# Zhangwenyao1/DreamVLA

Measured on AMD Instinct MI355X. Metric: train samples/sec (CALVIN ABC->D, seq_len=7), higher is better.
Workload: dtype bf16

## Files before the change

dreamvla_amd/csrc/gemm.hip:

```cpp
#include <stdlib.h>

#include <mutex>
#include "gemm_phase.h"
#include "gemm_skinny.h"

namespace dvla_gemm {
#define DVLA_EXTERN_REG(CF, AT, BT, DBG) extern template void launch_one<CF, AT, BT, DBG>(const GemmKArgs&, int, hipStream_t);
#define DVLA_EXTERN_RING(RC, AT, BT, EPI) extern template void launch_ring_one<RC, AT, BT, EPI>(const GemmKArgs&, int, hipStream_t);
#define DVLA_EXTERN_PHASE(AT, BT, EPI, DBG) extern template void launch_phase_one<AT, BT, EPI, DBG>(const GemmKArgs&, int, hipStream_t);
#include "gemm_inst_list.h"
#undef DVLA_EXTERN_REG
#undef DVLA_EXTERN_RING
#undef DVLA_EXTERN_PHASE
}

using namespace dvla_gemm;
namespace {
struct KsumJob { const float* partial; void* out; int64_t len; int rows; int out_bf16; unsigned main_blocks; };
__device__ __forceinline__ bool ksum_tail(const KsumJob& kj) {
  if (blockIdx.x < kj.main_blocks) return false;
  __shared__ float red[16][16];
  const int cl = threadIdx.x & 15, part = threadIdx.x >> 4;
  const int64_t c = (int64_t)(blockIdx.x - kj.main_blocks) * 16 + cl;
  float s = 0.f;
  if (c < kj.len)
#pragma unroll 4
    for (int r = part; r < kj.rows; r += 16) s += kj.partial[(int64_t)r * kj.len + c];
  red[part][cl] = s;
  __syncthreads();
  if (part == 0 && c < kj.len) {
    float tot = 0.f;
#pragma unroll
    for (int q = 0; q < 16; ++q) tot += red[q][cl];
    if (kj.out_bf16) reinterpret_cast<bf16_t*>(kj.out)[c] = f2bf(tot); else reinterpret_cast<float*>(kj.out)[c] = tot;
  }
  return true;
}
__global__ void splitk_reduce_vec_kernel(const float* __restrict__ ws, void* C, int64_t ldc, int c_f32, int accumulate,
                                         int64_t M, int64_t N, int splits, KsumJob kj) {
  if (ksum_tail(kj)) return;
  const int64_t octs = N >> 3;
  const int64_t idx = (int64_t)blockIdx.x * blockDim.x + threadIdx.x;
  if (idx >= M * octs) return;
  const int64_t m = idx / octs, n = (idx - m * octs) << 3;
  const int64_t MN = M * N;
  const float* src = ws + m * N + n;
  float4 a = make_float4(0.f, 0.f, 0.f, 0.f), b = a;
  for (int k = 0; k < splits; ++k) {
    const float4 x = *reinterpret_cast<const float4*>(src + (int64_t)k * MN);
    const float4 y = *reinterpret_cast<const float4*>(src + (int64_t)k * MN + 4);
    a.x += x.x; a.y += x.y; a.z += x.z; a.w += x.w; b.x += y.x; b.y += y.y; b.z += y.z; b.w += y.w;
  }
  if (c_f32) {
    float* c = reinterpret_cast<float*>(C) + m * ldc + n;
    if (accumulate) {
      const float4 o0 = *reinterpret_cast<const float4*>(c), o1 = *reinterpret_cast<const float4*>(c + 4);
      a.x += o0.x; a.y += o0.y; a.z += o0.z; a.w += o0.w; b.x += o1.x; b.y += o1.y; b.z += o1.z; b.w += o1.w;
    }
    *reinterpret_cast<float4*>(c) = a;
    *reinterpret_cast<float4*>(c + 4) = b;
  } else {
    *reinterpret_cast<uint4*>(reinterpret_cast<bf16_t*>(C) + m * ldc + n) =
        make_uint4(pack2bf(a.x, a.y), pack2bf(a.z, a.w), pack2bf(b.x, b.y), pack2bf(b.z, b.w));
  }
}
struct SplitEpi {
  const void* bias; int bias_f32; int act;
  const bf16_t* residual; int64_t ld_res; int64_t res_rows;
};
__global__ void splitk_reduce_epi_kernel(const float* __restrict__ ws, void* C, int64_t ldc, int c_f32, int64_t M, int64_t N,
                                         int splits, SplitEpi e) {
  const int64_t octs = N >> 3;
  const int64_t idx = (int64_t)blockIdx.x * blockDim.x + threadIdx.x;
  if (idx >= M * octs) return;
  const int64_t m = idx / octs, n = (idx - m * octs) << 3;
  const int64_t MN = M * N;
  const float* src = ws + m * N + n;
  float v[8] = {0.f, 0.f, 0.f, 0.f, 0.f, 0.f, 0.f, 0.f};
  for (int k = 0; k < splits; ++k) {
    const float4 x = *reinterpret_cast<const float4*>(src + (int64_t)k * MN);
    const float4 y = *reinterpret_cast<const float4*>(src + (int64_t)k * MN + 4);
    v[0] += x.x; v[1] += x.y; v[2] += x.z; v[3] += x.w; v[4] += y.x; v[5] += y.y; v[6] += y.z; v[7] += y.w;
  }
  if (e.bias) {
    if (e.bias_f32) {
      const float4 b0 = *reinterpret_cast<const float4*>(reinterpret_cast<const float*>(e.bias) + n);
      const float4 b1 = *reinterpret_cast<const float4*>(reinterpret_cast<const float*>(e.bias) + n + 4);
      v[0] += b0.x; v[1] += b0.y; v[2] += b0.z; v[3] += b0.w; v[4] += b1.x; v[5] += b1.y; v[6] += b1.z; v[7] += b1.w;
    } else {
      const uint4 b = *reinterpret_cast<const uint4*>(reinterpret_cast<const bf16_t*>(e.bias) + n);
      const uint32_t w[4] = {b.x, b.y, b.z, b.w};
#pragma unroll
      for (int i = 0; i < 4; ++i) { v[2 * i] += __uint_as_float(w[i] << 16); v[2 * i + 1] += __uint_as_float(w[i] & 0xffff0000u); }
    }
  }
  act_fwd8(v, e.act);
// ... 109 lines not shown
static std::mutex g_sk_mu;
static int g_streamk = -1;
static bool streamk_enabled() {
  if (g_streamk < 0) { const char* e = getenv("DVLA_GEMM_STREAMK"); g_streamk = (e && e[0] == '0') ? 0 : 1; }
  return g_streamk == 1;
}
static bool sk_scratch(hipStream_t stream, int groups, float** slabs, unsigned** flags) {
  if (!streamk_enabled()) return false;
  int dev = 0;
  if (hipGetDevice(&dev) != hipSuccess) return false;
  std::lock_guard<std::mutex> lk(g_sk_mu);
  for (int i = 0; i < g_sk_n; ++i)
    if (g_sk[i].dev == dev && g_sk[i].stream == stream && g_sk[i].groups >= groups) { *slabs = g_sk[i].slabs; *flags = g_sk[i].flags; return true; }
  if (g_sk_n == 16) return false;
  hipStreamCaptureStatus st = hipStreamCaptureStatusNone;
  if (hipStreamIsCapturing(stream, &st) != hipSuccess) { (void)hipGetLastError(); return false; }
  if (st != hipStreamCaptureStatusNone) return false;
  SkScratch e{dev, stream, nullptr, nullptr, groups};
  if (hipMalloc(reinterpret_cast<void**>(&e.slabs), (size_t)groups * PCfg::BM * PCfg::BN * 4) != hipSuccess) { (void)hipGetLastError(); return false; }
  if (hipMalloc(reinterpret_cast<void**>(&e.flags), (size_t)(groups + 1) * 4) != hipSuccess) { (void)hipGetLastError(); (void)hipFree(e.slabs); return false; }
  if (hipMemsetAsync(e.flags, 0, (size_t)(groups + 1) * 4, stream) != hipSuccess) { (void)hipGetLastError(); (void)hipFree(e.slabs); (void)hipFree(e.flags); return false; }
  g_sk[g_sk_n++] = e;
  *slabs = e.slabs; *flags = e.flags;
  return true;
}
inline int streamk_tiles(int64_t tiles, int cus, bool full = false) {
  if (cus % 16 != 0) return 0;
  const int64_t groups = cus / 16, st = (tiles + 15) / 16;
  if (st < groups || st % groups == 0) return 0;
  if (full) return (int)st;
  const int64_t dp_rounds = st / groups - 1;
  return (int)(st - dp_rounds * groups);
}
void launch_phase(GemmKArgs& a, int combo, int split_k, hipStream_t stream, int stream_k = 0) {
  set_tiles<PCfg::BM, PCfg::BN, PCfg::GH>(a);
  a.sk_tiles = 0;
  if (a.K % PCfg::BKS != 0) {
    if (a.ksum_op != 0) launch_phase_one<true, true, EPI_F32, 128 | 8192>(a, split_k, stream);
    else launch_phase_one<true, true, EPI_F32, 128>(a, split_k, stream);
    return;
  }
  if (a.ksum_op != 0) {
    launch_phase_one<true, true, EPI_F32, 8192>(a, split_k, stream);
    return;
  }
  if (stream_k && split_k == 1 && a.ksum_op == 0) {
    const int groups = num_cus();
    const int r = streamk_tiles((int64_t)a.tiles_m * a.tiles_n, groups, stream_k == 2);
    if (r > 0 && sk_scratch(stream, groups, &a.sk_slabs, &a.sk_flags)) a.sk_tiles = r;
  }
  switch (combo) {
    case 0: launch_phase_epi<false, false>(a, split_k, stream); break;
    case 1: launch_phase_epi<false, true>(a, split_k, stream); break;
    case 2: launch_phase_epi<true, false>(a, split_k, stream); break;
    default: launch_phase_epi<true, true>(a, split_k, stream); break;
  }
}
template <class RC>
bool ring_ok(const GemmKArgs& a, int combo) {
  if (!a.a_vec || !a.b_vec || !a.c_vec || !a.aux_vec || !a.epi_vec) return false;
  if (a.K < RC::BKS || a.K % RC::BKS != 0 || a.k_per_split % RC::BKS != 0 || (a.N & 63) != 0) return false;
  if ((int64_t)((a.M + RC::BM - 1) / RC::BM) * ((a.N + RC::BN - 1) / RC::BN) * a.split_k >= (1ll << 30)) return false;
  if (a.M < RC::BM || a.N < RC::BN) return false;
  if ((combo & 2) && (a.M % RC::BM != 0)) return false;
  if ((combo & 1) && (a.N % RC::BN != 0)) return false;
  const int64_t a_far = (int64_t)(((combo & 2) ? RC::BKS : RC::BM) - 1) * a.lda * 2 + 2 * (int64_t)((combo & 2) ? RC::BM : RC::BKS);
  const int64_t b_far = (int64_t)(((combo & 1) ? RC::BKS : RC::BN) - 1) * a.ldb * 2 + 2 * (int64_t)((combo & 1) ? RC::BN : RC::BKS);
  if (a_far >= (1ll << 32) || b_far >= (1ll << 32)) return false;
  return true;
}

bool phase_tail(const GemmKArgs& a, int combo) {
  return a.K % PCfg::BKS != 0 && combo == 3 && epi_class(a) == EPI_F32 && a.K % 16 == 0 && a.K >= 2 * PCfg::BKS;
}
bool phase_ok(const GemmKArgs& a, int combo) {
  if (phase_tail(a, combo)) {
    GemmKArgs b = a;
    b.K = a.K - a.K % PCfg::BKS;
    if (!ring_ok<PCfg>(b, combo)) return false;
  } else if (!ring_ok<PCfg>(a, combo)) return false;
  const int64_t a_rows = (combo & 2) ? a.K : a.M, b_rows = (combo & 1) ? a.K : a.N;
  return a_rows * a.lda * 2 < (1ll << 32) && b_rows * a.ldb * 2 < (1ll << 32);
}

inline double fill(int64_t tiles, int64_t slots) {
  const int64_t rounds = (tiles + slots - 1) / slots;
  return (double)tiles / (double)(rounds * slots);
}

}

static bool launch_phase_experiment(int idx, GemmKArgs& a, int split_k, hipStream_t stream) {
  switch (idx) {
    case 0: launch_phase_one<false, false, 0, 7424>(a, split_k, stream); return true;
    case 1: launch_phase_one<false, false, 0, 7488>(a, split_k, stream); return true;
    case 2: launch_phase_one<false, false, 0, 3328>(a, split_k, stream); return true;
    case 3: launch_phase_one<false, false, 0, 256>(a, split_k, stream); return true;
    case 4: launch_phase_one<false, false, 0, 32768>(a, split_k, stream); return true;
    case 5: launch_phase_one<false, false, 0, 16384 | 65536>(a, split_k, stream); return true;
    case 6: launch_phase_one<false, false, 0, 16384 | 65536 | 131072>(a, split_k, stream); return true;
    case 7: launch_phase_one<false, false, 0, 16384>(a, split_k, stream); return true;
    default: return false;
  }
}

static int g_last_variant = 0;
extern "C" int dvla_last_gemm_variant(void) { return g_last_variant; }
extern "C" void dvla_set_gemm_variant(int v) { g_gemm_variant = v; }
extern "C" void dvla_set_gemm_schedule(int oversubscribe, int stream_k) {
  if (oversubscribe >= 1) dvla_gemm::gemm_oversubscribe() = oversubscribe > 16 ? 16 : oversubscribe;
  if (stream_k >= 0) g_streamk = stream_k ? 1 : 0;
}

extern "C" void dvla_get_gemm_schedule(int* oversubscribe, int* stream_k) {
  if (oversubscribe) *oversubscribe = dvla_gemm::gemm_oversubscribe();
  if (stream_k) *stream_k = streamk_enabled() ? 1 : 0;
}

extern "C" int64_t dvla_gemm_ksum_partial_rows(int32_t split_k) {
  const int64_t fused = (int64_t)(split_k > 1 ? split_k : 1) * dvla_gemm::KSUM_PARTS * 4, fallback = dvla_colsum_partial_rows();
  return fused > fallback ? fused : fallback;
}

extern "C" int dvla_gemm_bf16(const dvla_gemm_params* q, void* stream_) {
  hipStream_t stream = reinterpret_cast<hipStream_t>(stream_);
  if (!q || !q->A || !q->B || !q->C) return DVLA_ERR_ARG;
  if (q->M < 0 || q->N < 0 || q->K < 0) return DVLA_ERR_ARG;
  if (q->M == 0 || q->N == 0) return DVLA_OK;
  if (q->accumulate && q->c_dtype != DVLA_DT_F32) return DVLA_ERR_ARG;
  if (q->dropout_p < 0.f || q->dropout_p >= 1.f) return DVLA_ERR_ARG;
  const int split_k = q->split_k > 1 ? q->split_k : 1;
  const bool split_epi = split_k > 1 && (q->bias || q->act || q->residual);
  if (split_k > 1) {
    if (!q->workspace || q->preact || q->dact_aux || q->dropout_p > 0.f) return DVLA_ERR_ARG;
    if (split_epi) {
      if (q->accumulate || q->ksum_operand != 0) return DVLA_ERR_ARG;
      const bool c_ok = q->c_dtype == DVLA_DT_F32 ? ((q->ldc % 4 == 0) && aligned(q->C, 16)) : ((q->ldc % 8 == 0) && aligned(q->C, 16));
      if ((q->N & 7) != 0 || !aligned(q->workspace, 16) || !c_ok || (q->bias && !aligned(q->bias, 16)) ||
          (q->residual && !((q->ld_res % 8 == 0) && aligned(q->residual, 16))))
        return DVLA_ERR_UNSUPPORTED;
    }
  }
  if (q->ksum_operand != 0) {
    if ((q->ksum_operand != 1 && q->ksum_operand != 2) || !q->ksum || !q->ksum_workspace) return DVLA_ERR_ARG;
    if (q->ksum_dtype != DVLA_DT_F32 && q->ksum_dtype != DVLA_DT_BF16) return DVLA_ERR_ARG;
  }
  GemmKArgs a;
  a.sk_tiles = 0; a.sk_slabs = nullptr; a.sk_flags = nullptr;
  a.ksum_ws = q->ksum_workspace; a.ksum_op = 0;
  a.ksum_parts = KSUM_PARTS;
  a.a_ln = q->a_layernorm != 0; a.a_ln_eps = q->a_ln_eps;
  a.A = reinterpret_cast<const bf16_t*>(q->A); a.lda = q->lda;
  a.B = reinterpret_cast<const bf16_t*>(q->B); a.ldb = q->ldb;
  a.C = q->C; a.ldc = q->ldc; a.c_f32 = (q->c_dtype == DVLA_DT_F32);
  a.M = q->M; a.N = q->N; a.K = q->K;
  a.bias = q->bias; a.bias_f32 = (q->bias_dtype == DVLA_DT_F32);
  a.act = q->act;
  a.preact = reinterpret_cast<bf16_t*>(q->preact); a.ld_preact = q->ld_preact;
  a.dact_aux = reinterpret_cast<const bf16_t*>(q->dact_aux); a.ld_dact = q->ld_dact; a.dact = q->dact;
  a.has_drop = q->dropout_p > 0.f;
  a.drop_scale = a.has_drop ? 1.0f / (1.0f - q->dropout_p) : 1.0f;
  {
    double thr = (double)q->dropout_p * 4294967296.0;
    a.drop_thr = thr >= 4294967295.0 ? 4294967295u : (uint32_t)thr;
  }
  a.seed_lo = q->seed_lo; a.seed_hi = q->seed_hi;
  a.residual = reinterpret_cast<const bf16_t*>(q->residual); a.ld_res = q->ld_res; a.res_rows = q->res_rows;
  a.accumulate = q->accumulate;
  a.split_k = split_k; a.workspace = reinterpret_cast<float*>(q->workspace);
  {
    int64_t nkt = (q->K + BK - 1) / BK;
    int64_t per = (nkt + split_k - 1) / split_k;
    a.k_per_split = per * BK;
  }
  a.a_vec = (q->lda % 8 == 0) && aligned(q->A, 16);
  a.b_vec = (q->ldb % 8 == 0) && aligned(q->B, 16);
  a.c_vec = a.c_f32 ? ((q->ldc % 4 == 0) && aligned(q->C, 16)) : ((q->ldc % 8 == 0) && aligned(q->C, 16));
  a.aux_vec = 1;
  if (q->preact && !((q->ld_preact % 8 == 0) && aligned(q->preact, 16))) a.aux_vec = 0;
  if (q->dact_aux && !((q->ld_dact % 8 == 0) && aligned(q->dact_aux, 16))) a.aux_vec = 0;
  if (q->residual && !((q->ld_res % 8 == 0) && aligned(q->residual, 16))) a.aux_vec = 0;
  if (split_epi) { a.bias = nullptr; a.act = 0; a.residual = nullptr; }
  a.epi_vec = 1;
  if (q->bias && !aligned(q->bias, 16)) a.epi_vec = 0;
  if (split_k > 1 && ((q->N & 3) != 0 || !aligned(q->workspace, 16))) a.epi_vec = 0;

  const int combo = (q->a_trans ? 2 : 0) | (q->b_trans ? 1 : 0);
  int variant = gemm_variant();
  if (variant >= 100) variant %= 100;
  {
    int choice = 0;
    if (a.a_ln && !(skinny_ok(a, combo, split_k) && skinny_ln_ok(a))) return DVLA_ERR_UNSUPPORTED;
    if ((variant == 0 || variant == 11 || a.a_ln) && skinny_ok(a, combo, split_k)) {
      choice = 11;
    } else if (variant == 0) {
      const double ns = (double)(a.k_per_split < a.K ? a.k_per_split : a.K) / 32.0;
      const int slots = num_cus();
      double best = 1e30;
      auto consider = [&](int c, int64_t bm, int64_t bn, int wg_per_cu, double fixed_us, double stage_us) {
        const int64_t items = ((q->M + bm - 1) / bm) * ((q->N + bn - 1) / bn) * split_k;
        const int64_t rounds = (items + (int64_t)slots * wg_per_cu - 1) / ((int64_t)slots * wg_per_cu);
        const double t = (double)rounds * (fixed_us + stage_us * ns);
        if (t < best) { best = t; choice = c; }
      };
      if (ring_ok<RCfgS>(a, combo)) consider(3, 128, 128, 2, 2.9, 0.58);
      if (ring_ok<RCfgM64>(a, combo)) consider(4, 256, 128, 1, 3.6, 0.49);
      if (ring_ok<RCfgL>(a, combo)) consider(1, 256, 256, 1, 5.8, 0.85);
      if (phase_ok(a, combo)) {
        consider(5, 256, 256, 1, 6.6, 0.775);
        const int64_t tiles = ((q->M + 255) / 256) * ((q->N + 255) / 256);
        if (split_k == 1 && streamk_enabled() && streamk_tiles(tiles, slots) > 0) {
          const double t = (double)tiles / slots * (6.6 + 0.775 * ns) + 18.0;
          if (t < best) { best = t; choice = 6; }
        }
      }
    } else if (variant == 4 && ring_ok<RCfgL>(a, combo)) choice = 1;
    else if (variant == 6 && ring_ok<RCfgS>(a, combo)) choice = 3;
    else if (variant == 7 && ring_ok<RCfgM64>(a, combo)) choice = 4;
    else if (variant == 8 && phase_ok(a, combo)) choice = 5;
    else if (variant == 9 && phase_ok(a, combo)) choice = 6;
    else if (variant == 10 && phase_ok(a, combo)) choice = 7;
    else if (variant > 80 && variant < 90 && combo == 0 && phase_ok(a, combo)) choice = 80 + (variant - 80);
    else if (variant >= 40 && variant < 48 && combo == 0 && phase_ok(a, combo) && epi_class(a) == EPI_P0) choice = variant;
    const bool phase_choice = choice == 5 || choice == 6 || choice == 7;
    const bool ksum_fused = q->ksum_operand != 0 && epi_class(a) == EPI_F32 &&
                            (choice == 1 || choice == 3 || choice == 4 || (phase_choice && combo == 3));
    if (ksum_fused) {
      a.ksum_op = q->ksum_operand;
      if (phase_choice) {
        const int64_t other = q->ksum_operand == 1 ? (q->N + PCfg::BN - 1) / PCfg::BN : (q->M + PCfg::BM - 1) / PCfg::BM;
        a.ksum_parts = KSUM_PARTS * (int)(other < 4 ? other : 4);
      }
    }
    switch (choice) {
      case 1: launch_ring<RCfgL>(a, combo, split_k, stream); break;
      case 3: launch_ring<RCfgS>(a, combo, split_k, stream); break;
      case 4: launch_ring<RCfgM64>(a, combo, split_k, stream); break;
      case 5: launch_phase(a, combo, split_k, stream); break;
      case 6: launch_phase(a, combo, split_k, stream, 1); break;
      case 7: launch_phase(a, combo, split_k, stream, 2); break;
      case 11: launch_skinny(a, stream); break;
      case 81: case 83: case 84: case 85: case 86: case 88: case 89:
        set_tiles<PCfg::BM, PCfg::BN, PCfg::GH>(a);
        if (epi_class(a) != EPI_P0) return DVLA_ERR_UNSUPPORTED;
        if (choice == 81) launch_phase_one<false, false, 0, 1>(a, split_k, stream);
        else if (choice == 83) launch_phase_one<false, false, 0, 3>(a, split_k, stream);
        else if (choice == 84) launch_phase_one<false, false, 0, 4>(a, split_k, stream);
        else if (choice == 85) launch_phase_one<false, false, 0, 16>(a, split_k, stream);
        else if (choice == 86) launch_phase_one<false, false, 0, 32>(a, split_k, stream);
        else if (choice == 88) launch_phase_one<false, false, 0, 16448>(a, split_k, stream);
        else launch_phase_one<false, false, 0, 64>(a, split_k, stream);
        break;
      default:
        if (choice >= 40 && choice < 48) {
          set_tiles<PCfg::BM, PCfg::BN, PCfg::GH>(a);
          a.sk_tiles = 0;
          if (launch_phase_experiment(choice - 40, a, split_k, stream)) break;
        }
        launch_cfg<CfgS>(a, combo, split_k, stream); break;
    }
    g_last_variant = choice == 11 ? 11 : choice == 1 ? 4 : choice == 3 ? 6 : choice == 4 ? 7 : choice == 5 ? 8
                   : (choice == 6 || choice == 7) ? (a.sk_tiles > 0 ? (choice == 6 ? 9 : 10) : 8) : choice >= 80 ? choice : 2;
  }
  int rc = dvla_check_launch();
  if (rc != DVLA_OK) return rc;
  KsumJob kj{nullptr, nullptr, 0, 0, 0, 0xffffffffu};
  if (q->ksum_operand != 0) {
    const int64_t len = q->ksum_operand == 1 ? q->M : q->N;
    if (a.ksum_op != 0) {
      if (split_k > 1) kj = KsumJob{a.ksum_ws, q->ksum, len, split_k * a.ksum_parts, q->ksum_dtype == DVLA_DT_BF16, 0u};
      else rc = dvla_reduce_partial_rows(a.ksum_ws, split_k * a.ksum_parts, len, len, q->ksum, q->ksum_dtype == DVLA_DT_BF16, stream);
    } else {
      const bool kmajor = q->ksum_operand == 1 ? q->a_trans != 0 : q->b_trans != 0;
      if (!kmajor) return DVLA_ERR_UNSUPPORTED;
      rc = dvla_colsum_dt(q->ksum_operand == 1 ? q->A : q->B, q->ksum_operand == 1 ? q->lda : q->ldb, q->K, len, q->ksum,
                          q->ksum_dtype, q->ksum_workspace, stream_);
    }
    if (rc != DVLA_OK) return rc;
  }
  if (split_k > 1) {
    const int64_t total = q->M * q->N;
    const bool vec = (q->N & 7) == 0 && aligned(a.workspace, 16) && aligned(q->C, 16) &&
                     (a.c_f32 ? (q->ldc & 3) == 0 : (q->ldc & 7) == 0);
    const unsigned main_blocks = (unsigned)(((vec ? total / 8 : total) + 255) / 256);
    const unsigned tail_blocks = kj.partial ? (unsigned)((kj.len + 15) / 16) : 0u;
    if (kj.partial) kj.main_blocks = main_blocks;
    if (split_epi) {
      SplitEpi e;
      e.bias = q->bias; e.bias_f32 = q->bias_dtype == DVLA_DT_F32; e.act = q->act;
      e.residual = reinterpret_cast<const bf16_t*>(q->residual); e.ld_res = q->ld_res; e.res_rows = q->res_rows;
      hipLaunchKernelGGL(splitk_reduce_epi_kernel, dim3(main_blocks), dim3(256), 0, stream, a.workspace, q->C, q->ldc, a.c_f32, q->M,
                         q->N, split_k, e);
    } else if (vec)
      hipLaunchKernelGGL(splitk_reduce_vec_kernel, dim3(main_blocks + tail_blocks), dim3(256), 0, stream,
                         a.workspace, q->C, q->ldc, a.c_f32, q->accumulate, q->M, q->N, split_k, kj);
    else
      hipLaunchKernelGGL(splitk_reduce_kernel, dim3(main_blocks + tail_blocks), dim3(256), 0, stream,
                         a.workspace, q->C, q->ldc, a.c_f32, q->accumulate, q->M, q->N, split_k, kj);
    rc = dvla_check_launch();
  }
  return rc;
}
```

dreamvla_amd/csrc/gemm_inst_list.h:

```cpp
DVLA_EXTERN_REG(CfgS, false, false, 0)
DVLA_EXTERN_REG(CfgS, false, true, 0)
DVLA_EXTERN_REG(CfgS, true, false, 0)
DVLA_EXTERN_REG(CfgS, true, true, 0)
DVLA_EXTERN_RING(RCfgL, false, false, 0)
DVLA_EXTERN_RING(RCfgL, false, false, 1)
DVLA_EXTERN_RING(RCfgL, false, false, 2)
DVLA_EXTERN_RING(RCfgL, false, false, 3)
DVLA_EXTERN_RING(RCfgL, false, false, 4)
DVLA_EXTERN_RING(RCfgL, false, false, 5)
DVLA_EXTERN_RING(RCfgL, false, false, 6)
DVLA_EXTERN_RING(RCfgL, false, false, 7)
DVLA_EXTERN_RING(RCfgL, false, true, 0)
DVLA_EXTERN_RING(RCfgL, false, true, 1)
DVLA_EXTERN_RING(RCfgL, false, true, 2)
DVLA_EXTERN_RING(RCfgL, false, true, 3)
DVLA_EXTERN_RING(RCfgL, false, true, 4)
DVLA_EXTERN_RING(RCfgL, false, true, 5)
DVLA_EXTERN_RING(RCfgL, false, true, 6)
DVLA_EXTERN_RING(RCfgL, false, true, 7)
DVLA_EXTERN_RING(RCfgL, true, false, 0)
DVLA_EXTERN_RING(RCfgL, true, false, 1)
DVLA_EXTERN_RING(RCfgL, true, false, 2)
DVLA_EXTERN_RING(RCfgL, true, false, 3)
DVLA_EXTERN_RING(RCfgL, true, false, 4)
// ... 42 lines not shown
DVLA_EXTERN_RING(RCfgS, true, true, 7)
DVLA_EXTERN_RING(RCfgM64, false, false, 0)
DVLA_EXTERN_RING(RCfgM64, false, false, 1)
DVLA_EXTERN_RING(RCfgM64, false, false, 2)
DVLA_EXTERN_RING(RCfgM64, false, false, 3)
DVLA_EXTERN_RING(RCfgM64, false, false, 4)
DVLA_EXTERN_RING(RCfgM64, false, false, 5)
DVLA_EXTERN_RING(RCfgM64, false, false, 6)
DVLA_EXTERN_RING(RCfgM64, false, false, 7)
DVLA_EXTERN_RING(RCfgM64, false, true, 0)
DVLA_EXTERN_RING(RCfgM64, false, true, 1)
DVLA_EXTERN_RING(RCfgM64, false, true, 2)
DVLA_EXTERN_RING(RCfgM64, false, true, 3)
DVLA_EXTERN_RING(RCfgM64, false, true, 4)
DVLA_EXTERN_RING(RCfgM64, false, true, 5)
DVLA_EXTERN_RING(RCfgM64, false, true, 6)
DVLA_EXTERN_RING(RCfgM64, false, true, 7)
DVLA_EXTERN_RING(RCfgM64, true, false, 0)
DVLA_EXTERN_RING(RCfgM64, true, false, 1)
DVLA_EXTERN_RING(RCfgM64, true, false, 2)
DVLA_EXTERN_RING(RCfgM64, true, false, 3)
DVLA_EXTERN_RING(RCfgM64, true, false, 4)
DVLA_EXTERN_RING(RCfgM64, true, false, 5)
DVLA_EXTERN_RING(RCfgM64, true, false, 6)
DVLA_EXTERN_RING(RCfgM64, true, false, 7)
DVLA_EXTERN_RING(RCfgM64, true, true, 0)
DVLA_EXTERN_RING(RCfgM64, true, true, 1)
DVLA_EXTERN_RING(RCfgM64, true, true, 2)
DVLA_EXTERN_RING(RCfgM64, true, true, 3)
DVLA_EXTERN_RING(RCfgM64, true, true, 4)
DVLA_EXTERN_RING(RCfgM64, true, true, 5)
DVLA_EXTERN_RING(RCfgM64, true, true, 6)
DVLA_EXTERN_RING(RCfgM64, true, true, 7)
DVLA_EXTERN_PHASE(false, false, 0, 0)
DVLA_EXTERN_PHASE(false, false, 1, 0)
DVLA_EXTERN_PHASE(false, false, 2, 0)
DVLA_EXTERN_PHASE(false, false, 3, 0)
DVLA_EXTERN_PHASE(false, false, 4, 0)
DVLA_EXTERN_PHASE(false, false, 5, 0)
DVLA_EXTERN_PHASE(false, false, 6, 0)
DVLA_EXTERN_PHASE(false, false, 7, 0)
DVLA_EXTERN_PHASE(false, true, 0, 0)
DVLA_EXTERN_PHASE(false, true, 1, 0)
DVLA_EXTERN_PHASE(false, true, 2, 0)
DVLA_EXTERN_PHASE(false, true, 3, 0)
DVLA_EXTERN_PHASE(false, true, 4, 0)
DVLA_EXTERN_PHASE(false, true, 5, 0)
DVLA_EXTERN_PHASE(false, true, 6, 0)
DVLA_EXTERN_PHASE(false, true, 7, 0)
DVLA_EXTERN_PHASE(true, false, 0, 0)
DVLA_EXTERN_PHASE(true, false, 1, 0)
DVLA_EXTERN_PHASE(true, false, 2, 0)
DVLA_EXTERN_PHASE(true, false, 3, 0)
DVLA_EXTERN_PHASE(true, false, 4, 0)
DVLA_EXTERN_PHASE(true, false, 5, 0)
DVLA_EXTERN_PHASE(true, false, 6, 0)
DVLA_EXTERN_PHASE(true, false, 7, 0)
DVLA_EXTERN_PHASE(true, true, 0, 0)
DVLA_EXTERN_PHASE(true, true, 1, 0)
DVLA_EXTERN_PHASE(true, true, 2, 0)
DVLA_EXTERN_PHASE(true, true, 3, 0)
DVLA_EXTERN_PHASE(true, true, 4, 0)
DVLA_EXTERN_PHASE(true, true, 5, 0)
DVLA_EXTERN_PHASE(true, true, 6, 0)
DVLA_EXTERN_PHASE(true, true, 7, 0)
DVLA_EXTERN_PHASE(true, true, 6, 128)
DVLA_EXTERN_PHASE(true, true, 6, 8192)
DVLA_EXTERN_PHASE(true, true, 6, 8320)
DVLA_EXTERN_PHASE(false, false, 0, 1)
DVLA_EXTERN_PHASE(false, false, 0, 3)
DVLA_EXTERN_PHASE(false, false, 0, 4)
DVLA_EXTERN_PHASE(false, false, 0, 16)
DVLA_EXTERN_PHASE(false, false, 0, 32)
DVLA_EXTERN_PHASE(false, false, 0, 64)
DVLA_EXTERN_PHASE(false, false, 0, 7424)
DVLA_EXTERN_PHASE(false, false, 0, 7488)
DVLA_EXTERN_PHASE(false, false, 0, 3328)
DVLA_EXTERN_PHASE(false, false, 0, 256)
DVLA_EXTERN_PHASE(false, false, 0, 16384)
DVLA_EXTERN_PHASE(false, false, 0, 16448)
DVLA_EXTERN_PHASE(false, false, 0, 32768)
DVLA_EXTERN_PHASE(false, false, 0, 81920)
DVLA_EXTERN_PHASE(false, false, 0, 212992)
```

Measured before the change: 229.4.

## Add 256x128 phase-pipelined persistent GEMM kernel and route heuristic to it

```diff
diff --git a/dreamvla_amd/csrc/gemm.hip b/dreamvla_amd/csrc/gemm.hip
--- a/dreamvla_amd/csrc/gemm.hip
+++ b/dreamvla_amd/csrc/gemm.hip
@@ -2,16 +2,19 @@
 
 #include <mutex>
 #include "gemm_phase.h"
+#include "gemm_phase_h.h"
 #include "gemm_skinny.h"
 
 namespace dvla_gemm {
 #define DVLA_EXTERN_REG(CF, AT, BT, DBG) extern template void launch_one<CF, AT, BT, DBG>(const GemmKArgs&, int, hipStream_t);
 #define DVLA_EXTERN_RING(RC, AT, BT, EPI) extern template void launch_ring_one<RC, AT, BT, EPI>(const GemmKArgs&, int, hipStream_t);
 #define DVLA_EXTERN_PHASE(AT, BT, EPI, DBG) extern template void launch_phase_one<AT, BT, EPI, DBG>(const GemmKArgs&, int, hipStream_t);
+#define DVLA_EXTERN_PHASE_H(AT, BT, EPI, DBG) extern template void launch_phase_h_one<AT, BT, EPI, DBG>(const GemmKArgs&, int, hipStream_t);
 #include "gemm_inst_list.h"
 #undef DVLA_EXTERN_REG
 #undef DVLA_EXTERN_RING
 #undef DVLA_EXTERN_PHASE
+#undef DVLA_EXTERN_PHASE_H
 }
 
 using namespace dvla_gemm;
@@ -287,6 +290,47 @@
   const int64_t a_rows = (combo & 2) ? a.K : a.M, b_rows = (combo & 1) ? a.K : a.N;
   return a_rows * a.lda * 2 < (1ll << 32) && b_rows * a.ldb * 2 < (1ll << 32);
 }
+
+bool phase_h_tail(const GemmKArgs& a, int combo) {
+  return a.K % PCfgH::BKS != 0 && combo == 3 && epi_class(a) == EPI_F32 && a.K % 16 == 0 && a.K >= 2 * PCfgH::BKS;
+}
+bool phase_h_ok(const GemmKArgs& a, int combo) {
+  const int ec = epi_class(a);
+  if (ec == EPI_GEN || combo == 2 || (combo == 3 && ec != EPI_F32)) return false;
+  if (phase_h_tail(a, combo)) {
+    GemmKArgs b = a;
+    b.K = a.K - a.K % PCfgH::BKS;
+    if (!ring_ok<PCfgH>(b, combo)) return false;
+  } else if (!ring_ok<PCfgH>(a, combo)) return false;
+  const int64_t a_rows = (combo & 2) ? a.K : a.M, b_rows = (combo & 1) ? a.K : a.N;
+  return a_rows * a.lda * 2 < (1ll << 32) && b_rows * a.ldb * 2 < (1ll << 32);
+}
+template <bool AT, bool BT>
+void launch_phase_h_epi(const GemmKArgs& a, int split_k, hipStream_t stream) {
+  switch (epi_class(a)) {
+    case EPI_P0: launch_phase_h_one<AT, BT, EPI_P0, 0>(a, split_k, stream); break;
+    case EPI_P_ERF: launch_phase_h_one<AT, BT, EPI_P_ERF, 0>(a, split_k, stream); break;
+    case EPI_P_TANH: launch_phase_h_one<AT, BT, EPI_P_TANH, 0>(a, split_k, stream); break;
+    case EPI_A0: launch_phase_h_one<AT, BT, EPI_A0, 0>(a, split_k, stream); break;
+    case EPI_A_ERF: launch_phase_h_one<AT, BT, EPI_A_ERF, 0>(a, split_k, stream); break;
+    case EPI_A_TANH: launch_phase_h_one<AT, BT, EPI_A_TANH, 0>(a, split_k, stream); break;
+    default: launch_phase_h_one<AT, BT, EPI_F32, 0>(a, split_k, stream); break;
+  }
+}
+void launch_phase_h(GemmKArgs& a, int combo, int split_k, hipStream_t stream) {
+  set_tiles<PCfgH::BM, PCfgH::BN, PCfgH::GH>(a);
+  a.sk_tiles = 0;
+  if (combo == 3) {
+    const bool tail = a.K % PCfgH::BKS != 0;
+    if (a.ksum_op != 0) { if (tail) launch_phase_h_one<true, true, EPI_F32, 128 | 8192>(a, split_k, stream); else launch_phase_h_one<true, true, EPI_F32, 8192>(a, split_k, stream); }
+    else { if (tail) launch_phase_h_one<true, true, EPI_F32, 128>(a, split_k, stream); else launch_phase_h_one<true, true, EPI_F32, 0>(a, split_k, stream); }
+    return;
+  }
+  if (combo == 0) launch_phase_h_epi<false, false>(a, split_k, stream);
+  else launch_phase_h_epi<false, true>(a, split_k, stream);
+}
+
+constexpr double PH_FIXED_US = 4.0, PH_STAGE_US = 0.42;
 
 inline double fill(int64_t tiles, int64_t slots) {
   const int64_t rounds = (tiles + slots - 1) / slots;
@@ -410,6 +454,7 @@
       };
       if (ring_ok<RCfgS>(a, combo)) consider(3, 128, 128, 2, 2.9, 0.58);
       if (ring_ok<RCfgM64>(a, combo)) consider(4, 256, 128, 1, 3.6, 0.49);
+      if (phase_h_ok(a, combo)) consider(8, 256, 128, 1, PH_FIXED_US, PH_STAGE_US);
       if (ring_ok<RCfgL>(a, combo)) consider(1, 256, 256, 1, 5.8, 0.85);
       if (phase_ok(a, combo)) {
         consider(5, 256, 256, 1, 6.6, 0.775);
@@ -421,19 +466,21 @@
       }
     } else if (variant == 4 && ring_ok<RCfgL>(a, combo)) choice = 1;
     else if (variant == 6 && ring_ok<RCfgS>(a, combo)) choice = 3;
-    else if (variant == 7 && ring_ok<RCfgM64>(a, combo)) choice = 4;
+    else if (variant == 7 && phase_h_ok(a, combo)) choice = 8;
+    else if ((variant == 7 || variant == 17) && ring_ok<RCfgM64>(a, combo)) choice = 4;
     else if (variant == 8 && phase_ok(a, combo)) choice = 5;
     else if (variant == 9 && phase_ok(a, combo)) choice = 6;
     else if (variant == 10 && phase_ok(a, combo)) choice = 7;
     else if (variant > 80 && variant < 90 && combo == 0 && phase_ok(a, combo)) choice = 80 + (variant - 80);
     else if (variant >= 40 && variant < 48 && combo == 0 && phase_ok(a, combo) && epi_class(a) == EPI_P0) choice = variant;
-    const bool phase_choice = choice == 5 || choice == 6 || choice == 7;
+    const bool phase_choice = choice == 5 || choice == 6 || choice == 7 || choice == 8;
     const bool ksum_fused = q->ksum_operand != 0 && epi_class(a) == EPI_F32 &&
                             (choice == 1 || choice == 3 || choice == 4 || (phase_choice && combo == 3));
     if (ksum_fused) {
       a.ksum_op = q->ksum_operand;
       if (phase_choice) {
-        const int64_t other = q->ksum_operand == 1 ? (q->N + PCfg::BN - 1) / PCfg::BN : (q->M + PCfg::BM - 1) / PCfg::BM;
+        const int64_t bn = choice == 8 ? PCfgH::BN : PCfg::BN;
+        const int64_t other = q->ksum_operand == 1 ? (q->N + bn - 1) / bn : (q->M + PCfg::BM - 1) / PCfg::BM;
         a.ksum_parts = KSUM_PARTS * (int)(other < 4 ? other : 4);
       }
     }
@@ -444,6 +491,7 @@
       case 5: launch_phase(a, combo, split_k, stream); break;
       case 6: launch_phase(a, combo, split_k, stream, 1); break;
       case 7: launch_phase(a, combo, split_k, stream, 2); break;
+      case 8: launch_phase_h(a, combo, split_k, stream); break;
       case 11: launch_skinny(a, stream); break;
       case 81: case 83: case 84: case 85: case 86: case 88: case 89:
         set_tiles<PCfg::BM, PCfg::BN, PCfg::GH>(a);
@@ -464,7 +512,7 @@
         }
         launch_cfg<CfgS>(a, combo, split_k, stream); break;
     }
-    g_last_variant = choice == 11 ? 11 : choice == 1 ? 4 : choice == 3 ? 6 : choice == 4 ? 7 : choice == 5 ? 8
+    g_last_variant = choice == 11 ? 11 : choice == 1 ? 4 : choice == 3 ? 6 : choice == 4 ? 17 : choice == 8 ? 7 : choice == 5 ? 8
                    : (choice == 6 || choice == 7) ? (a.sk_tiles > 0 ? (choice == 6 ? 9 : 10) : 8) : choice >= 80 ? choice : 2;
   }
   int rc = dvla_check_launch();
diff --git a/dreamvla_amd/csrc/gemm_inst/phaseh_NN_e0.hip b/dreamvla_amd/csrc/gemm_inst/phaseh_NN_e0.hip
--- /dev/null
+++ b/dreamvla_amd/csrc/gemm_inst/phaseh_NN_e0.hip
@@ -0,0 +1,2 @@
+#include "../gemm_phase_h.h"
+namespace dvla_gemm { template void launch_phase_h_one<false, false, 0, 0>(const GemmKArgs&, int, hipStream_t); }
diff --git a/dreamvla_amd/csrc/gemm_inst/phaseh_NN_e1.hip b/dreamvla_amd/csrc/gemm_inst/phaseh_NN_e1.hip
--- /dev/null
+++ b/dreamvla_amd/csrc/gemm_inst/phaseh_NN_e1.hip
@@ -0,0 +1,2 @@
+#include "../gemm_phase_h.h"
+namespace dvla_gemm { template void launch_phase_h_one<false, false, 1, 0>(const GemmKArgs&, int, hipStream_t); }
diff --git a/dreamvla_amd/csrc/gemm_inst/phaseh_NN_e2.hip b/dreamvla_amd/csrc/gemm_inst/phaseh_NN_e2.hip
--- /dev/null
+++ b/dreamvla_amd/csrc/gemm_inst/phaseh_NN_e2.hip
@@ -0,0 +1,2 @@
+#include "../gemm_phase_h.h"
+namespace dvla_gemm { template void launch_phase_h_one<false, false, 2, 0>(const GemmKArgs&, int, hipStream_t); }
diff --git a/dreamvla_amd/csrc/gemm_inst/phaseh_NN_e3.hip b/dreamvla_amd/csrc/gemm_inst/phaseh_NN_e3.hip
--- /dev/null
+++ b/dreamvla_amd/csrc/gemm_inst/phaseh_NN_e3.hip
@@ -0,0 +1,2 @@
+#include "../gemm_phase_h.h"
+namespace dvla_gemm { template void launch_phase_h_one<false, false, 3, 0>(const GemmKArgs&, int, hipStream_t); }
diff --git a/dreamvla_amd/csrc/gemm_inst/phaseh_NN_e4.hip b/dreamvla_amd/csrc/gemm_inst/phaseh_NN_e4.hip
--- /dev/null
+++ b/dreamvla_amd/csrc/gemm_inst/phaseh_NN_e4.hip
@@ -0,0 +1,2 @@
+#include "../gemm_phase_h.h"
+namespace dvla_gemm { template void launch_phase_h_one<false, false, 4, 0>(const GemmKArgs&, int, hipStream_t); }
diff --git a/dreamvla_amd/csrc/gemm_inst/phaseh_NN_e5.hip b/dreamvla_amd/csrc/gemm_inst/phaseh_NN_e5.hip
--- /dev/null
+++ b/dreamvla_amd/csrc/gemm_inst/phaseh_NN_e5.hip
@@ -0,0 +1,2 @@
+#include "../gemm_phase_h.h"
+namespace dvla_gemm { template void launch_phase_h_one<false, false, 5, 0>(const GemmKArgs&, int, hipStream_t); }
diff --git a/dreamvla_amd/csrc/gemm_inst/phaseh_NN_e6.hip b/dreamvla_amd/csrc/gemm_inst/phaseh_NN_e6.hip
--- /dev/null
+++ b/dreamvla_amd/csrc/gemm_inst/phaseh_NN_e6.hip
@@ -0,0 +1,2 @@
+#include "../gemm_phase_h.h"
+namespace dvla_gemm { template void launch_phase_h_one<false, false, 6, 0>(const GemmKArgs&, int, hipStream_t); }
diff --git a/dreamvla_amd/csrc/gemm_inst/phaseh_NT_e0.hip b/dreamvla_amd/csrc/gemm_inst/phaseh_NT_e0.hip
--- /dev/null
+++ b/dreamvla_amd/csrc/gemm_inst/phaseh_NT_e0.hip
@@ -0,0 +1,2 @@
+#include "../gemm_phase_h.h"
+namespace dvla_gemm { template void launch_phase_h_one<false, true, 0, 0>(const GemmKArgs&, int, hipStream_t); }
diff --git a/dreamvla_amd/csrc/gemm_inst/phaseh_NT_e1.hip b/dreamvla_amd/csrc/gemm_inst/phaseh_NT_e1.hip
--- /dev/null
+++ b/dreamvla_amd/csrc/gemm_inst/phaseh_NT_e1.hip
@@ -0,0 +1,2 @@
+#include "../gemm_phase_h.h"
+namespace dvla_gemm { template void launch_phase_h_one<false, true, 1, 0>(const GemmKArgs&, int, hipStream_t); }
diff --git a/dreamvla_amd/csrc/gemm_inst/phaseh_NT_e2.hip b/dreamvla_amd/csrc/gemm_inst/phaseh_NT_e2.hip
--- /dev/null
+++ b/dreamvla_amd/csrc/gemm_inst/phaseh_NT_e2.hip
@@ -0,0 +1,2 @@
+#include "../gemm_phase_h.h"
+namespace dvla_gemm { template void launch_phase_h_one<false, true, 2, 0>(const GemmKArgs&, int, hipStream_t); }
diff --git a/dreamvla_amd/csrc/gemm_inst/phaseh_NT_e3.hip b/dreamvla_amd/csrc/gemm_inst/phaseh_NT_e3.hip
--- /dev/null
+++ b/dreamvla_amd/csrc/gemm_inst/phaseh_NT_e3.hip
@@ -0,0 +1,2 @@
+#include "../gemm_phase_h.h"
+namespace dvla_gemm { template void launch_phase_h_one<false, true, 3, 0>(const GemmKArgs&, int, hipStream_t); }
diff --git a/dreamvla_amd/csrc/gemm_inst/phaseh_NT_e4.hip b/dreamvla_amd/csrc/gemm_inst/phaseh_NT_e4.hip
--- /dev/null
+++ b/dreamvla_amd/csrc/gemm_inst/phaseh_NT_e4.hip
@@ -0,0 +1,2 @@
+#include "../gemm_phase_h.h"
+namespace dvla_gemm { template void launch_phase_h_one<false, true, 4, 0>(const GemmKArgs&, int, hipStream_t); }
diff --git a/dreamvla_amd/csrc/gemm_inst/phaseh_NT_e5.hip b/dreamvla_amd/csrc/gemm_inst/phaseh_NT_e5.hip
--- /dev/null
+++ b/dreamvla_amd/csrc/gemm_inst/phaseh_NT_e5.hip
@@ -0,0 +1,2 @@
+#include "../gemm_phase_h.h"
+namespace dvla_gemm { template void launch_phase_h_one<false, true, 5, 0>(const GemmKArgs&, int, hipStream_t); }
diff --git a/dreamvla_amd/csrc/gemm_inst/phaseh_NT_e6.hip b/dreamvla_amd/csrc/gemm_inst/phaseh_NT_e6.hip
--- /dev/null
+++ b/dreamvla_amd/csrc/gemm_inst/phaseh_NT_e6.hip
@@ -0,0 +1,2 @@
+#include "../gemm_phase_h.h"
+namespace dvla_gemm { template void launch_phase_h_one<false, true, 6, 0>(const GemmKArgs&, int, hipStream_t); }
diff --git a/dreamvla_amd/csrc/gemm_inst/phaseh_TT_e6.hip b/dreamvla_amd/csrc/gemm_inst/phaseh_TT_e6.hip
--- /dev/null
+++ b/dreamvla_amd/csrc/gemm_inst/phaseh_TT_e6.hip
@@ -0,0 +1,5 @@
+#include "../gemm_phase_h.h"
+namespace dvla_gemm {
+template void launch_phase_h_one<true, true, 6, 0>(const GemmKArgs&, int, hipStream_t);
+template void launch_phase_h_one<true, true, 6, 128>(const GemmKArgs&, int, hipStream_t);
+}
diff --git a/dreamvla_amd/csrc/gemm_inst/phaseh_TT_e6_ksum.hip b/dreamvla_amd/csrc/gemm_inst/phaseh_TT_e6_ksum.hip
--- /dev/null
+++ b/dreamvla_amd/csrc/gemm_inst/phaseh_TT_e6_ksum.hip
@@ -0,0 +1,5 @@
+#include "../gemm_phase_h.h"
+namespace dvla_gemm {
+template void launch_phase_h_one<true, true, 6, 8192>(const GemmKArgs&, int, hipStream_t);
+template void launch_phase_h_one<true, true, 6, 8320>(const GemmKArgs&, int, hipStream_t);
+}
diff --git a/dreamvla_amd/csrc/gemm_inst_list.h b/dreamvla_amd/csrc/gemm_inst_list.h
--- a/dreamvla_amd/csrc/gemm_inst_list.h
+++ b/dreamvla_amd/csrc/gemm_inst_list.h
@@ -148,3 +148,21 @@
 DVLA_EXTERN_PHASE(false, false, 0, 32768)
 DVLA_EXTERN_PHASE(false, false, 0, 81920)
 DVLA_EXTERN_PHASE(false, false, 0, 212992)
+DVLA_EXTERN_PHASE_H(false, false, 0, 0)
+DVLA_EXTERN_PHASE_H(false, false, 1, 0)
+DVLA_EXTERN_PHASE_H(false, false, 2, 0)
+DVLA_EXTERN_PHASE_H(false, false, 3, 0)
+DVLA_EXTERN_PHASE_H(false, false, 4, 0)
+DVLA_EXTERN_PHASE_H(false, false, 5, 0)
+DVLA_EXTERN_PHASE_H(false, false, 6, 0)
+DVLA_EXTERN_PHASE_H(false, true, 0, 0)
+DVLA_EXTERN_PHASE_H(false, true, 1, 0)
+DVLA_EXTERN_PHASE_H(false, true, 2, 0)
+DVLA_EXTERN_PHASE_H(false, true, 3, 0)
+DVLA_EXTERN_PHASE_H(false, true, 4, 0)
+DVLA_EXTERN_PHASE_H(false, true, 5, 0)
+DVLA_EXTERN_PHASE_H(false, true, 6, 0)
+DVLA_EXTERN_PHASE_H(true, true, 6, 0)
+DVLA_EXTERN_PHASE_H(true, true, 6, 128)
+DVLA_EXTERN_PHASE_H(true, true, 6, 8192)
+DVLA_EXTERN_PHASE_H(true, true, 6, 8320)
diff --git a/dreamvla_amd/csrc/gemm_phase_h.h b/dreamvla_amd/csrc/gemm_phase_h.h
--- /dev/null
+++ b/dreamvla_amd/csrc/gemm_phase_h.h
@@ -0,0 +1,291 @@
+#pragma once
+#include "gemm_phase.h"
+
+namespace dvla_gemm {
+
+struct PCfgH {
+  static constexpr int BM = 256, BN = 128, BKS = 64, GH = 4, NT = 512;
+  static constexpr int A_BYTES = BM * BKS * 2, B_BYTES = BN * BKS * 2;
+  static constexpr int NI = 3;
+  static constexpr int B_BASE = NI * A_BYTES;
+  static constexpr int SMEM_BYTES = NI * (A_BYTES + B_BYTES);
+  static constexpr int CPWA = 4, CPWB = 2;
+  static constexpr int NPW = CPWA + CPWB;
+  static constexpr int UP_TO_LOAD1 = 3, UP_TO_LOAD2 = 6;
+  static_assert(A_BYTES / 1024 == 8 * CPWA && B_BYTES / 1024 == 8 * CPWB, "pieces per wave");
+  static_assert(SMEM_BYTES <= 160 * 1024, "LDS budget");
+};
+
+template <bool A_T, bool B_T, int EPI, int DBG = 0>
+__global__ __launch_bounds__(PCfgH::NT) __attribute__((amdgpu_waves_per_eu(2, 2)))
+void gemm_phase_kernel_h(GemmKArgs p) {
+  constexpr int BM = PCfgH::BM, BN = PCfgH::BN, BKS = PCfgH::BKS, CPWA = PCfgH::CPWA, CPWB = PCfgH::CPWB;
+  constexpr bool TAIL = (DBG & 128) != 0;
+  constexpr bool KSUM = EPI == EPI_F32 && (DBG & 8192) != 0;
+  static_assert((DBG & ~(128 | 8192)) == 0, "production builds only");
+  static_assert(!TAIL || (A_T && B_T), "partial K-tiles: k-major operands only");
+  static_assert(EPI != EPI_GEN, "the generic class runs on the ring kernel");
+  extern __shared__ __attribute__((aligned(16))) char smem[];
+  const int t = threadIdx.x;
+  const int lane = t & 63;
+  const int wave = __builtin_amdgcn_readfirstlane(t >> 6);
+  const int grp = wave >> 2, wc = wave & 3;
+  const int wr = wc >> 1, wn = wc & 1;
+
+  const int nitems = p.tiles_m * p.tiles_n * p.split_k;
+  const int grid = gridDim.x;
+  const int perm = [&] {
+    const int q8 = grid >> 3, r8 = grid & 7, xcd = (int)(blockIdx.x & 7), idx = (int)(blockIdx.x >> 3);
+    return (xcd < r8 ? xcd * (q8 + 1) : r8 * (q8 + 1) + (xcd - r8) * q8) + idx;
+  }();
+  struct Seg { int m0, n0, k_begin, ns, split; };
+  auto tail_steps = [&](const Seg& sg) -> int {
+    if constexpr (!TAIL) return 4;
+    const int64_t k_last = (int64_t)sg.k_begin + (int64_t)(sg.ns - 1) * BKS;
+    const int64_t left = p.K - k_last;
+    return left >= BKS ? 4 : (int)(left / 16);
+  };
+  Seg c_seg = {0, 0, 0, 0, 0};
+  int c_it = -1;
+  bool c_ok = false;
+  auto seg_cached = [&](int it, Seg& sg) -> bool {
+    if (it != c_it) {
+      c_it = it;
+      const int id = it * grid + perm;
+      c_ok = id < nitems;
+      if (c_ok) {
+        const RingItem w = ring_item<PCfgH>(p, id);
+        c_seg.m0 = (int)w.m0; c_seg.n0 = (int)w.n0; c_seg.k_begin = (int)w.k_begin; c_seg.ns = w.ns; c_seg.split = w.split;
+      }
+    }
+    sg = c_seg;
+    return c_ok;
+  };
+  const uint32_t smem_base = (uint32_t)(uintptr_t)(__attribute__((address_space(3))) char*)smem;
+
+  uint32_t srcA[CPWA];
+  uint32_t srcB[CPWB];
+  int itA = 0, ktA = 0, nkA = 0, nA = 0; bool liveA = false;
+  int itB = 0, ktB = 0, nkB = 0, nB = 0; bool liveB = false;
+  int tvA = 4, tvB = 4;
+  const uint32_t stepA = (uint32_t)(2 * (A_T ? (int64_t)BKS * p.lda : (int64_t)BKS));
+  const uint32_t stepB = (uint32_t)(2 * (B_T ? (int64_t)BKS * p.ldb : (int64_t)BKS));
+  const char* kbA = reinterpret_cast<const char*>(p.A);
+  const char* kbB = reinterpret_cast<const char*>(p.B);
+  uint32_t m0A = smem_base + (uint32_t)(wave * (CPWA * 1024));
+  uint32_t m0B = smem_base + (uint32_t)(PCfgH::B_BASE + wave * (CPWB * 1024));
+  auto openA = [&](int it) {
+    Seg w;
+    liveA = seg_cached(it, w);
+    if (!liveA) return;
+    nkA = w.ns; ktA = 0; tvA = tail_steps(w);
+    kbA = reinterpret_cast<const char*>(p.A);
+#pragma unroll
+    for (int i = 0; i < CPWA; ++i)
+      srcA[i] = (uint32_t)(reinterpret_cast<const char*>(dma_src<A_T, BM, BKS>(p.A, p.lda, w.m0, p.M, w.k_begin, wave * CPWA + i, lane)) -
+                           reinterpret_cast<const char*>(p.A));
+  };
+  auto openB = [&](int it) {
+    Seg w;
+    liveB = seg_cached(it, w);
+    if (!liveB) return;
+    nkB = w.ns; ktB = 0; tvB = tail_steps(w);
+    kbB = reinterpret_cast<const char*>(p.B);
+#pragma unroll
+    for (int i = 0; i < CPWB; ++i)
+      srcB[i] = (uint32_t)(reinterpret_cast<const char*>(dma_src<B_T, BN, BKS>(p.B, p.ldb, w.n0, p.N, w.k_begin, wave * CPWB + i, lane)) -
+                           reinterpret_cast<const char*>(p.B));
+  };
+  auto tail_back = [&](int c, int rows_div8, int tv, int64_t ld) -> uint32_t {
+    const int k_local = (64 * c + lane) / rows_div8;
+    return k_local >= 16 * tv ? (uint32_t)(2 * (int64_t)k_local * ld) : 0u;
+  };
+  auto pieceA = [&](auto ic) {
+    constexpr int i = decltype(ic)::value;
+    uint32_t off = srcA[i];
+    if constexpr (TAIL) { if (tvA < 4 && ktA == nkA - 1) off -= tail_back(wave * CPWA + i, BM / 8, tvA, p.lda); }
+    glds16s_lean<i * 1024>(kbA, off, (uint32_t)__builtin_amdgcn_readfirstlane((int)m0A));
+  };
+  auto doneA = [&]() {
+    nA = nA == PCfgH::NI - 1 ? 0 : nA + 1;
+    kbA += stepA;
+    m0A = nA == 0 ? m0A - (uint32_t)((PCfgH::NI - 1) * PCfgH::A_BYTES) : m0A + (uint32_t)PCfgH::A_BYTES;
+    if (++ktA == nkA) openA(++itA);
+  };
+  auto pieceB = [&](auto ic) {
+    constexpr int i = decltype(ic)::value;
+    uint32_t off = srcB[i];
+    if constexpr (TAIL) { if (tvB < 4 && ktB == nkB - 1) off -= tail_back(wave * CPWB + i, BN / 8, tvB, p.ldb); }
+    glds16s_lean<i * 1024>(kbB, off, (uint32_t)__builtin_amdgcn_readfirstlane((int)m0B));
+  };
+  auto doneB = [&]() {
+    nB = nB == PCfgH::NI - 1 ? 0 : nB + 1;
+    kbB += stepB;
+    m0B = nB == 0 ? m0B - (uint32_t)((PCfgH::NI - 1) * PCfgH::B_BYTES) : m0B + (uint32_t)PCfgH::B_BYTES;
+    if (++ktB == nkB) openB(++itB);
+  };
+  auto issueA = [&]() -> bool {
+    if (!liveA) return false;
+    static_for<CPWA>([&](auto ic) { pieceA(ic); });
+    doneA();
+    return true;
+  };
+  auto issueB = [&]() -> bool {
+    if (!liveB) return false;
+    static_for<CPWB>([&](auto ic) { pieceB(ic); });
+    doneB();
+    return true;
+  };
+  auto emit = [&](auto h_c, auto ia, auto ib) {
+    constexpr int H = decltype(h_c)::value;
+    __builtin_amdgcn_sched_barrier(0);
+    if (ia) { pieceA(std::integral_constant<int, 2 * H>{}); pieceA(std::integral_constant<int, 2 * H + 1>{}); if (H == 1) doneA(); }
+    if (ib) { pieceB(std::integral_constant<int, H>{}); if (H == 1) doneB(); }
+    __builtin_amdgcn_sched_barrier(0);
+  };
+
+  openA(0); openB(0);
+  issueA();
+  issueB();
+  const bool a1 = issueA();
+  const bool b1 = issueB();
+  if (a1 && b1) wait_vmcnt<PCfgH::NPW>(); else wait_vmcnt<0>();
+  __builtin_amdgcn_s_barrier();
+
+  int ua = 0;
+  for (int it = 0;; ++it) {
+    Seg w;
+    if (!seg_cached(it, w)) break;
+    w.m0 = __builtin_amdgcn_readfirstlane(w.m0); w.n0 = __builtin_amdgcn_readfirstlane(w.n0);
+    w.split = __builtin_amdgcn_readfirstlane(w.split);
+    const int seg_ns = w.ns;
+    const int seg_tv = __builtin_amdgcn_readfirstlane(tail_steps(w));
+    f32x16 acc[2][2];
+#pragma unroll
+    for (int i = 0; i < 2; ++i)
+#pragma unroll
+      for (int j = 0; j < 2; ++j)
+#pragma unroll
+        for (int r = 0; r < 16; ++r) acc[i][j][r] = 0.f;
+    float ksa[2] = {0.f, 0.f};
+    const int ks_c = !KSUM ? 0 : p.ksum_op == 1 ? w.n0 / BN : w.m0 / BM;
+    int ks_cnt = (KSUM && ks_c * KSUM_PARTS < p.ksum_parts) ? ks_c : -1;
+    if (grp == 1) __builtin_amdgcn_s_barrier();
+    __builtin_amdgcn_sched_barrier(0);
+
+    auto load = [&](auto h_c, const char* bufA, const char* bufB, bf16x8 (&fa)[2][2], bf16x8 (&fb)[2][2]) {
+      constexpr int H = decltype(h_c)::value;
+#pragma unroll
+      for (int s = 0; s < 2; ++s) {
+#pragma unroll
+        for (int i = 0; i < 2; ++i) fb[i][s] = ring_frag<B_T, BN, BKS>(bufB, wn * 64 + i * 32, 2 * H + s, lane);
+#pragma unroll
+        for (int j = 0; j < 2; ++j) fa[j][s] = ring_frag<A_T, BM, BKS>(bufA, grp * 128 + wr * 64 + j * 32, 2 * H + s, lane);
+      }
+    };
+    auto mfma = [&](bf16x8 (&fa)[2][2], bf16x8 (&fb)[2][2]) {
+      __builtin_amdgcn_s_setprio(1);
+#pragma unroll
+      for (int s = 0; s < 2; ++s)
+#pragma unroll
+        for (int i = 0; i < 2; ++i)
+#pragma unroll
+          for (int j = 0; j < 2; ++j) acc[i][j] = __builtin_amdgcn_mfma_f32_32x32x16_bf16(fb[i][s], fa[j][s], acc[i][j], 0, 0, 0);
+      __builtin_amdgcn_s_setprio(0);
+      __builtin_amdgcn_sched_barrier(0);
+    };
+    auto after_reads = [&](auto h_c, int kt, bf16x8 (&fa)[2][2], bf16x8 (&fb)[2][2]) {
+      constexpr int H = decltype(h_c)::value;
+      const int tv_now = (TAIL && kt == seg_ns - 1) ? seg_tv : 4;
+      if constexpr (TAIL) {
+        if (tv_now < 4) {
+#pragma unroll
+          for (int s = 0; s < 2; ++s)
+            if (2 * H + s >= tv_now) { fa[0][s] = bf16x8{0, 0, 0, 0, 0, 0, 0, 0}; fa[1][s] = bf16x8{0, 0, 0, 0, 0, 0, 0, 0}; }
+        }
+        __builtin_amdgcn_sched_barrier(0);
+      }
+      if constexpr (KSUM) {
+        if (ks_cnt == 0 && p.ksum_op == 1) {
+          static_for<2>([&](auto sc) {
+            constexpr int s = decltype(sc)::value;
+            if (wn == s) { ksa[0] = ksum_add_sel(fa[0][s], 0x3f803f80u, ksa[0]); ksa[1] = ksum_add_sel(fa[1][s], 0x3f803f80u, ksa[1]); }
+          });
+        }
+        if (ks_cnt == 0 && p.ksum_op == 2) {
+          const int q = 2 * grp + wr;
+          static_for<2>([&](auto sc) {
+            constexpr int s = decltype(sc)::value;
+            if (q == 2 * H + s && 2 * H + s < tv_now) {
+              ksa[0] = ksum_add_sel(fb[0][s], 0x3f803f80u, ksa[0]); ksa[1] = ksum_add_sel(fb[1][s], 0x3f803f80u, ksa[1]);
+            }
+          });
+        }
+        if (H == 1) ks_cnt = ks_cnt > 0 ? ks_cnt - 1 : (ks_cnt == 0 ? p.ksum_parts / KSUM_PARTS - 1 : ks_cnt);
+        __builtin_amdgcn_sched_barrier(0);
+      }
+    };
+
+    auto kloop = [&](auto live_c) {
+      for (int kt = 0; kt < seg_ns; ++kt, ua = (ua == PCfgH::NI - 1 ? 0 : ua + 1)) {
+        const char* bufA = smem + ua * PCfgH::A_BYTES;
+        const char* bufB = smem + PCfgH::B_BASE + ua * PCfgH::B_BYTES;
+        bf16x8 fa[2][2], fb[2][2];
+        const bool after_epi = !TAIL && kt == 0 && it > 0;
+        const auto ia = live_or(live_c, liveA);
+        const auto ib = live_or(live_c, liveB);
+        emit(std::integral_constant<int, 0>{}, ia, ib);
+        load(std::integral_constant<int, 0>{}, bufA, bufB, fa, fb);
+        wait_lds();
+        __builtin_amdgcn_sched_barrier(0);
+        after_reads(std::integral_constant<int, 0>{}, kt, fa, fb);
+        __builtin_amdgcn_s_barrier();
+        mfma(fa, fb);
+        __builtin_amdgcn_s_barrier();
+        emit(std::integral_constant<int, 1>{}, ia, ib);
+        load(std::integral_constant<int, 1>{}, bufA, bufB, fa, fb);
+        if (grp == 1 && !after_epi) { if (ia && ib) wait_vmcnt<PCfgH::UP_TO_LOAD2>(); else wait_vmcnt<0>(); }
+        wait_lds();
+        __builtin_amdgcn_sched_barrier(0);
+        after_reads(std::integral_constant<int, 1>{}, kt, fa, fb);
+        __builtin_amdgcn_s_barrier();
+        mfma(fa, fb);
+        if (!after_epi) { if (ia && ib) wait_vmcnt<PCfgH::NPW>(); else wait_vmcnt<0>(); }
+        __builtin_amdgcn_s_barrier();
+      }
+    };
+    if constexpr (!(TAIL && KSUM)) {
+      Seg nx;
+      const bool all_live = seg_cached(it + 1, nx) && nx.ns >= 2;
+      if (all_live) kloop(std::true_type{}); else kloop(std::false_type{});
+    } else {
+      kloop(std::false_type{});
+    }
+    if constexpr (KSUM) {
+      const int tc = p.ksum_op == 1 ? w.n0 / BN : w.m0 / BM;
+      if (ks_cnt >= 0 && p.ksum_op == 1) ksum_store<2, 2>(p, ksa, lane, w.split, wn, 2, (int64_t)w.m0 + grp * 128 + wr * 64, p.M, tc * KSUM_PARTS);
+      if (ks_cnt >= 0 && p.ksum_op == 2) ksum_store<2, 2>(p, ksa, lane, w.split, 2 * grp + wr, 4, (int64_t)w.n0 + wn * 64, p.N, tc * KSUM_PARTS);
+    }
+    if constexpr (!TAIL) wait_vmcnt<0>();
+    if (grp == 0) __builtin_amdgcn_s_barrier();
+    __builtin_amdgcn_sched_barrier(0);
+    int lane_e = lane;
+    asm volatile("" : "+v"(lane_e));
+    reg_epilogue<2, EPI>(p, acc, lane_e, (int64_t)w.m0 + grp * 128 + wr * 64, (int64_t)w.n0 + wn * 64, w.split);
+  }
+}
+
+template <bool A_T, bool B_T, int EPI, int DBG = 0>
+void launch_phase_h_one(const GemmKArgs& a, int split_k, hipStream_t stream) {
+  static bool attr_set = false;
+  auto kern = &gemm_phase_kernel_h<A_T, B_T, EPI, DBG>;
+  if (!attr_set) {
+    (void)hipFuncSetAttribute(reinterpret_cast<const void*>(kern), hipFuncAttributeMaxDynamicSharedMemorySize, PCfgH::SMEM_BYTES);
+    attr_set = true;
+  }
+  const int64_t items = (int64_t)a.tiles_m * a.tiles_n * split_k;
+  dim3 grid((unsigned)persistent_grid(items, (int64_t)num_cus()), 1, 1), block(PCfgH::NT, 1, 1);
+  hipLaunchKernelGGL(kern, grid, block, PCfgH::SMEM_BYTES, stream, a);
+}
+
+}
```

New measurement: 229.6 (median of 6 runs). No clear change (+0.1%).
